# LuoweiZhou/VLP

Measured on NVIDIA H100. Metric: image_text_samples_per_sec, higher is better.
Workload: dtype bf16

## Files before the change

### vlp_b200/csrc/api.cu

```cuda
#include "../../include/vlpk.h"

#include <cstdlib>
#include <cstring>

#include "attn.cuh"
#include "decode.cuh"
#include "gemm.cuh"
#include "head.cuh"
#include "host.cuh"
#include "optim.cuh"
#include "rowops.cuh"
#include "tables.cuh"

using namespace vlpk;
typedef __nv_bfloat16 bf16;

namespace {

inline cudaStream_t S(void* s) { return reinterpret_cast<cudaStream_t>(s); }

enum { SITE_ATTN = 0, SITE_HID1 = 1, SITE_HID2 = 2 };
inline uint64_t site_of(uint64_t layer_id, int site) { return layer_id * 8 + site; }

inline DropoutCfg mk_drop(const VlpkDropout* d, float p, uint64_t site) {
// ... 187 lines not shown
  VLPK_TRY(launch_attn_fwd(ad, st));
  VLPK_TRY(fwd_linear(Mq, H, H, a->ctx, H, w->wo, H, w->bo, a->t1, H, EPI_STORE, nullptr, 0, none, st));
  LnArgs ln;
  ln.M = Mq; ln.H = H;
  ln.t = static_cast<const bf16*>(a->t1); ln.res = static_cast<const bf16*>(x);
  ln.gamma = static_cast<const bf16*>(w->ln1_g); ln.beta = static_cast<const bf16*>(w->ln1_b);
  ln.y = static_cast<bf16*>(a->y1); ln.stats = reinterpret_cast<float2*>(a->stats1);
  ln.drop = mk_drop(drop, p_hidden, site_of(layer_id, SITE_HID1));
  return launch_ln_res_drop_fwd(ln, st);
}

int ffn_fwd_impl(const VlpkShape* s, const VlpkLayerWeights* w, VlpkLayerActs* a, float p_hidden, const VlpkDropout* drop,
                 uint64_t layer_id, cudaStream_t st) {
  const int H = s->H, I = s->I, M = s->B * s->Lq;
  const DropoutCfg none = make_dropout(0.f, 0, 0);
  VLPK_TRY(fwd_linear(M, I, H, a->y1, H, w->w1, H, w->b1, a->u, I, EPI_GELU, a->hmid, I, none, st));
  VLPK_TRY(fwd_linear(M, H, I, a->hmid, I, w->w2, I, w->b2, a->t2, H, EPI_STORE, nullptr, 0, none, st));
  LnArgs ln;
  ln.M = M; ln.H = H;
  ln.t = static_cast<const bf16*>(a->t2); ln.res = static_cast<const bf16*>(a->y1);
  ln.gamma = static_cast<const bf16*>(w->ln2_g); ln.beta = static_cast<const bf16*>(w->ln2_b);
  ln.y = static_cast<bf16*>(a->y); ln.stats = reinterpret_cast<float2*>(a->stats2);
  ln.drop = mk_drop(drop, p_hidden, site_of(layer_id, SITE_HID2));
  return launch_ln_res_drop_fwd(ln, st);
}

int ffn_bwd_impl(const VlpkShape* s, const VlpkLayerWeights* w, const VlpkLayerActs* a, const void* dy, void* dy1,
                 const VlpkLayerGrads* g, const VlpkBwdScratch* ws, float p_hidden, const VlpkDropout* drop, uint64_t layer_id,
                 cudaStream_t st) {
  VLPK_CHECK_ARG(s->Lq == s->Lkv, "ffn_bwd: training path requires Lq == Lkv");
  const int H = s->H, I = s->I, M = s->B * s->Lq;
  const bool hdrop = (drop != nullptr && p_hidden > 0.f);
  LnArgs l2;
  l2.M = M; l2.H = H;
  l2.t = static_cast<const bf16*>(a->t2); l2.res = static_cast<const bf16*>(a->y1);
  l2.gamma = static_cast<const bf16*>(w->ln2_g); l2.stats = reinterpret_cast<float2*>(a->stats2);
  l2.dy = static_cast<const bf16*>(dy);
  l2.dz = static_cast<bf16*>(ws->dz2);
  l2.dt = hdrop ? static_cast<bf16*>(ws->dt2) : nullptr;
  l2.dgamma = g->ln2_g; l2.dbeta = g->ln2_b; l2.dbias = g->b2;
  l2.drop = mk_drop(drop, p_hidden, site_of(layer_id, SITE_HID2));
  VLPK_TRY(launch_ln_res_drop_bwd(l2, st));
  const void* dt2 = hdrop ? ws->dt2 : ws->dz2;
  VLPK_TRY(linear_bwd_pair(
      st, [&](cudaStream_t q) { return wgrad_linear(M, H, I, dt2, H, a->hmid, I, g->w2, I, q); },
      [&](cudaStream_t q) {
        if (!deterministic()) return dgrad_linear(M, H, I, dt2, H, w->w2, I, ws->du, I, EPI_MUL, a->u, I, q, g->b1);
        VLPK_TRY(dgrad_linear(M, H, I, dt2, H, w->w2, I, ws->du, I, EPI_MUL, a->u, I, q));
        return launch_colsum(ws->du, I, M, I, g->b1, q);
      }));
  VLPK_TRY(linear_bwd_pair(
      st, [&](cudaStream_t q) { return wgrad_linear(M, I, H, ws->du, I, a->y1, H, g->w1, H, q); },
      [&](cudaStream_t q) { return dgrad_linear(M, I, H, ws->du, I, w->w1, H, dy1, H, EPI_ADD, ws->dz2, H, q); }));
  return wgrad_join(st);
}

int mha_bwd_impl(const VlpkShape* s, const VlpkLayerWeights* w, const void* x, const uint32_t* bits, int mask_rows,
                 const VlpkLayerActs* a, const void* dy1, void* dx, const VlpkLayerGrads* g, const VlpkBwdScratch* ws, float p_attn,
                 float p_hidden, const VlpkDropout* drop, uint64_t layer_id, cudaStream_t st) {
  VLPK_CHECK_ARG(s->Lq == s->Lkv, "mha_bwd: training path requires Lq == Lkv");
  const int H = s->H, M = s->B * s->Lq;
  const bool hdrop = (drop != nullptr && p_hidden > 0.f);
  LnArgs l1;
  l1.M = M; l1.H = H;
  l1.t = static_cast<const bf16*>(a->t1); l1.res = static_cast<const bf16*>(x);
  l1.gamma = static_cast<const bf16*>(w->ln1_g); l1.stats = reinterpret_cast<float2*>(a->stats1);
  l1.dy = static_cast<const bf16*>(dy1);
  l1.dz = static_cast<bf16*>(ws->dz1);
  l1.dt = hdrop ? static_cast<bf16*>(ws->dt1) : nullptr;
  l1.dgamma = g->ln1_g; l1.dbeta = g->ln1_b; l1.dbias = g->bo;
  l1.drop = mk_drop(drop, p_hidden, site_of(layer_id, SITE_HID1));
  VLPK_TRY(launch_ln_res_drop_bwd(l1, st));
  const void* dt1 = hdrop ? ws->dt1 : ws->dz1;
  VLPK_TRY(linear_bwd_pair(
      st, [&](cudaStream_t q) { return wgrad_linear(M, H, H, dt1, H, a->ctx, H, g->wo, H, q); },
      [&](cudaStream_t q) { return dgrad_linear(M, H, H, dt1, H, w->wo, H, ws->dctx, H, EPI_STORE, nullptr, 0, q); }));
  AttnDesc ad;
  ad.B = s->B; ad.heads = s->heads; ad.Lq = s->Lq; ad.Lkv = s->Lkv; ad.kv_slots = s->kv_slots;
  ad.q = a->qkv; ad.k = static_cast<const bf16*>(a->qkv) + H; ad.v = static_cast<const bf16*>(a->qkv) + 2 * H;
  ad.ld_q = 3 * H; ad.ld_kv = 3 * H;
  ad.o = a->ctx; ad.ld_o = H; ad.d_o = ws->dctx;
  ad.mask_bits = bits; ad.mask_rows = mask_rows; ad.lse = a->lse;
  ad.dq = ws->dqkv; ad.dk = static_cast<bf16*>(ws->dqkv) + H; ad.dv = static_cast<bf16*>(ws->dqkv) + 2 * H;
  ad.ld_dqkv = 3 * H;
  ad.drop = mk_drop(drop, p_attn, site_of(layer_id, SITE_ATTN));
  if (ad.drop.p > 0.f) ad.drop.bits = a->drop_attn;
  ad.dbias = g->bqkv;
  VLPK_TRY(launch_attn_bwd(ad, st));
  GemmDesc d;
  d.M = M; d.N = H; d.K = 3 * H;
  d.A = ws->dqkv; d.lda = 3 * H;
  d.b_mn = true; d.nseg = 3; d.b_seg_rows = H; d.ldb = H;
  d.B[0] = w->wq; d.B[1] = w->wk; d.B[2] = w->wv;
  d.D0 = dx; d.ldd0 = H;
  d.epi = EPI_ADD;
  d.aux = static_cast<const bf16*>(ws->dz1); d.ld_aux = H;
  VLPK_TRY(linear_bwd_pair(
      st, [&](cudaStream_t q) { return wgrad_linear(M, 3 * H, H, ws->dqkv, 3 * H, x, H, g->wqkv, H, q); },
      [&](cudaStream_t q) { return launch_gemm(d, q); }));
  return wgrad_join(st);
}

int layer_bwd_impl(const VlpkShape* s, const VlpkLayerWeights* w, const void* x, const uint32_t* bits, int mask_rows,
                   const VlpkLayerActs* a, const void* dy, void* dx, const VlpkLayerGrads* g, const VlpkBwdScratch* ws, float p_attn,
                   float p_hidden, const VlpkDropout* drop, uint64_t layer_id, cudaStream_t st) {
  VLPK_TRY(ffn_bwd_impl(s, w, a, dy, ws->dy1, g, ws, p_hidden, drop, layer_id, st));
  return mha_bwd_impl(s, w, x, bits, mask_rows, a, ws->dy1, dx, g, ws, p_attn, p_hidden, drop, layer_id, st);
}

__global__ void add_bf16_kernel(bf16* __restrict__ dst, const bf16* __restrict__ a, const bf16* __restrict__ b, long long n) {
  const long long i = (static_cast<long long>(blockIdx.x) * blockDim.x + threadIdx.x) * 8;
  if (i + 8 <= n) {
    const uint4 ua = *reinterpret_cast<const uint4*>(a + i), ub = *reinterpret_cast<const uint4*>(b + i);
    const uint32_t wa[4] = {ua.x, ua.y, ua.z, ua.w}, wb[4] = {ub.x, ub.y, ub.z, ub.w};
    uint32_t o[4];
#pragma unroll
    for (int j = 0; j < 4; ++j) {
      const float2 x = unpack_bf16x2(wa[j]), y = unpack_bf16x2(wb[j]);
      o[j] = pack_bf16x2(x.x + y.x, x.y + y.y);
    }
    *reinterpret_cast<uint4*>(dst + i) = make_uint4(o[0], o[1], o[2], o[3]);
  } else {
    for (long long k = i; k < n; ++k) dst[k] = __float2bfloat16_rn(__bfloat162float(a[k]) + __bfloat162float(b[k]));
  }
}

__global__ void relu_bwd_kernel(bf16* __restrict__ dpre, const bf16* __restrict__ dy, const bf16* __restrict__ y, long long M,
                                int N, long long lddy, long long ldy, float scale) {
  const long long i = (static_cast<long long>(blockIdx.x) * blockDim.x + threadIdx.x) * 8;
  if (i >= M * N) return;
  const long long r = i / N;
  const int c = static_cast<int>(i % N);
  const uint4 ud = *reinterpret_cast<const uint4*>(dy + r * lddy + c), uy = *reinterpret_cast<const uint4*>(y + r * ldy + c);
  const uint32_t wd[4] = {ud.x, ud.y, ud.z, ud.w}, wy[4] = {uy.x, uy.y, uy.z, uy.w};
  uint32_t o[4];
#pragma unroll
  for (int j = 0; j < 4; ++j) {
    const float2 d = unpack_bf16x2(wd[j]), v = unpack_bf16x2(wy[j]);
    o[j] = pack_bf16x2(v.x > 0.f ? d.x * scale : 0.f, v.y > 0.f ? d.y * scale : 0.f);
  }
  *reinterpret_cast<uint4*>(dpre + i) = make_uint4(o[0], o[1], o[2], o[3]);
}

}

#pragma GCC visibility push(default)
extern "C" {

int vlpk_version(void) { return VLPK_VERSION; }
int vlpk_debug_set_option(const char* name, int value) {
  VLPK_CHECK_ARG(name != nullptr, "set_option: null name");
  if (strcmp(name, "wgrad_stream") == 0) { g_wgrad_stream = value ? 1 : 0; return 0; }
  if (strcmp(name, "attn_tiled") == 0) { set_attn_tiled(value != 0); return 0; }
  set_error("set_option: unknown option '%s'", name);
  return -1;
}
int vlpk_debug_plan_gemm(int M, int N, int K, int a_mn, int b_mn, int nseg, int seg_rows, int epi, int bn, int splits, int* out2) {
  GemmDesc g;
  g.M = M; g.N = N; g.K = K;
  g.a_mn = a_mn != 0; g.b_mn = b_mn != 0;
  g.nseg = nseg; g.b_seg_rows = seg_rows;
  g.epi = epi; g.bn = bn; g.splits = splits;
  return plan_gemm(g, &out2[0], &out2[1]);
}
void vlpk_set_reserved_sms(int n) { set_reserved_sms(n); }
void vlpk_set_deterministic(int on) { set_deterministic(on != 0); }
const char* vlpk_last_error(void) { return get_error(); }

int vlpk_mask_pack(const void* mask, int dtype, int mode, int B, int rows, int kv, int64_t stride_b, int64_t stride_r, uint32_t* out,
                   void* stream) {
  VLPK_CHECK_ARG(mask != nullptr && out != nullptr, "mask_pack: null pointer");
  return launch_mask_pack(mask, dtype, mode, B, rows, kv, stride_b, stride_r, out, S(stream));
}

int vlpk_mask_synth(const int32_t* len_b, const int32_t* mode, int len_a, int B, int L, uint32_t* out, void* stream) {
  return launch_mask_synth(len_b, mode, len_a, B, L, out, S(stream));
}

int vlpk_linear_fwd(int M, int N, int K, const void* x, int64_t ldx, const void* w, int64_t ldw, const void* bias, void* y, int64_t ldy,
                    int act, const VlpkDropout* drop, uint64_t site, void* stream) {
  VLPK_CHECK_ARG(x && w && y, "linear_fwd: null pointer");
  VLPK_CHECK_ARG(act == VLPK_ACT_NONE || act == VLPK_ACT_RELU, "linear_fwd: act %d unsupported", act);
  const DropoutCfg dc = (act == VLPK_ACT_RELU && drop != nullptr) ? mk_drop(drop, drop->p, site) : make_dropout(0.f, 0, site);
  return fwd_linear(M, N, K, x, ldx, w, ldw, bias, y, ldy, act == VLPK_ACT_RELU ? EPI_RELU : EPI_STORE, nullptr, 0, dc, S(stream));
}

int vlpk_linear_bwd(int M, int N, int K, const void* x, int64_t ldx, const void* w, int64_t ldw, const void* y, int64_t ldy,
                    const void* dy, int64_t lddy, void* dpre, void* dx, int64_t lddx, float* dw, int64_t lddw, float* db, int act,
                    float p_drop, void* stream) {
  VLPK_CHECK_ARG(x && w && dy && dw, "linear_bwd: null pointer");
  cudaStream_t st = S(stream);
  const void* g = dy;
  int64_t ldg = lddy;
  if (act == VLPK_ACT_RELU) {
    VLPK_CHECK_ARG(y != nullptr && dpre != nullptr && N % 8 == 0, "linear_bwd: relu needs y, dpre and N %% 8 == 0");
    const long long n = static_cast<long long>(M) * N;
    LaunchScope scope(CAT_MISC, 6.0 * n, st);
    relu_bwd_kernel<<<static_cast<unsigned>((n / 8 + 255) / 256), 256, 0, st>>>(static_cast<bf16*>(dpre), static_cast<const bf16*>(dy),
                                                                             static_cast<const bf16*>(y), M, N, lddy, ldy,
                                                                             p_drop > 0.f ? 1.0f / (1.0f - p_drop) : 1.0f);
    VLPK_CUDA(cudaGetLastError());
    g = dpre;
    ldg = N;
  }
  if (db != nullptr) VLPK_TRY(launch_colsum(g, ldg, M, N, db, st));
  VLPK_TRY(wgrad_linear(M, N, K, g, ldg, x, ldx, dw, lddw, st));
  if (dx != nullptr) VLPK_TRY(dgrad_linear(M, N, K, g, ldg, w, ldw, dx, lddx, EPI_STORE, nullptr, 0, st));
  return 0;
}

static EmbedArgs mk_embed(int B, int L, int H, int R, int vis_input, const int64_t* ids, const int64_t* tt, const int64_t* pos,
                          const void* word_w, const void* pos_w, const void* type_w, const void* vis, const void* vpe,
                          const void* ln_g) {
  EmbedArgs a;
  a.B = B; a.L = L; a.H = H; a.R = R; a.vis_input = vis_input;
  a.ids = reinterpret_cast<const long long*>(ids);
  a.tt = reinterpret_cast<const long long*>(tt);
  a.pos = reinterpret_cast<const long long*>(pos);
  a.word = static_cast<const bf16*>(word_w); a.posw = static_cast<const bf16*>(pos_w); a.typew = static_cast<const bf16*>(type_w);
  a.vis = static_cast<const bf16*>(vis); a.vpe = static_cast<const bf16*>(vpe);
  a.gamma = static_cast<const bf16*>(ln_g);
  return a;
}

int vlpk_embed_fwd(int B, int L, int H, int R, int vis_input, const int64_t* ids, const int64_t* token_type, const int64_t* pos,
                   const void* word_w, const void* pos_w, const void* type_w, const void* vis, const void* vis_pe, const void* ln_g,
                   const void* ln_b, void* y, float* stats, const VlpkDropout* drop, uint64_t site, void* stream) {
  VLPK_CHECK_ARG(ids && word_w && pos_w && type_w && ln_g && ln_b && y, "embed_fwd: null pointer");
  EmbedArgs a = mk_embed(B, L, H, R, vis_input, ids, token_type, pos, word_w, pos_w, type_w, vis, vis_pe, ln_g);
  a.beta = static_cast<const bf16*>(ln_b);
  a.y = static_cast<bf16*>(y);
  a.stats = reinterpret_cast<float2*>(stats);
  a.drop = mk_drop(drop, drop ? drop->p : 0.f, site);
  return launch_embed_fwd(a, S(stream));
}

int vlpk_embed_bwd(int B, int L, int H, int R, int vis_input, const int64_t* ids, const int64_t* token_type, const int64_t* pos,
                   const void* word_w, const void* pos_w, const void* type_w, const void* vis, const void* vis_pe, const void* ln_g,
                   const float* stats, const void* dy, void* dz, float* d_ln_g, float* d_ln_b, const VlpkDropout* drop, uint64_t site,
                   void* stream) {
  VLPK_CHECK_ARG(ids && word_w && pos_w && type_w && ln_g && stats && dy && dz, "embed_bwd: null pointer");
  EmbedArgs a = mk_embed(B, L, H, R, vis_input, ids, token_type, pos, word_w, pos_w, type_w, vis, vis_pe, ln_g);
  a.stats = reinterpret_cast<float2*>(const_cast<float*>(stats));
  a.dy = static_cast<const bf16*>(dy);
  a.dz = static_cast<bf16*>(dz);
  a.dgamma = d_ln_g; a.dbeta = d_ln_b;
  a.drop = mk_drop(drop, drop ? drop->p : 0.f, site);
  return launch_embed_bwd(a, S(stream));
}

int vlpk_embed_tables_bwd(int B, int L, int H, int R, int vis_input, const int64_t* ids, const int64_t* token_type, const int64_t* pos,
                          const void* dz, int V, int P, int T, void* d_word, float* word_scratch, float* d_pos, float* d_type,
                          void* stream) {
  TableGradArgs a;
  a.B = B; a.L = L; a.H = H; a.R = R; a.vis_input = vis_input;
  a.V = V; a.P = P; a.T = T;
  a.ids = reinterpret_cast<const long long*>(ids);
  a.tt = reinterpret_cast<const long long*>(token_type);
  a.pos = reinterpret_cast<const long long*>(pos);
  a.dz = static_cast<const bf16*>(dz);
  a.d_word = static_cast<bf16*>(d_word);
  a.scratch = word_scratch; a.d_pos = d_pos; a.d_type = d_type;
  return launch_embed_tables_bwd(a, S(stream));
}

int vlpk_table_rows_add(int64_t n, const int64_t* ids, const int64_t* pos, const void* rows, int H, int V, int P, float scale, void* d_word,
                        float* scratch, int32_t* owner, float* d_pos, void* stream) {
  TableRowsArgs a;
  a.n = n; a.H = H; a.V = V; a.P = P; a.scale = scale;
  a.ids = reinterpret_cast<const long long*>(ids);
  a.pos = reinterpret_cast<const long long*>(pos);
  a.rows = static_cast<const bf16*>(rows);
  a.d_word = static_cast<bf16*>(d_word);
  a.scratch = scratch; a.owner = owner; a.d_pos = d_pos;
  return launch_table_rows_add(a, S(stream));
}

int vlpk_ln_res_drop_fwd(int64_t M, int H, const void* t, const void* res, const void* gamma, const void* beta, void* y, float* stats,
                         const VlpkDropout* drop, uint64_t site, void* stream) {
  VLPK_CHECK_ARG(t && gamma && beta && y, "ln_res_drop_fwd: null pointer");
  LnArgs a;
  a.M = M; a.H = H;
  a.t = static_cast<const bf16*>(t); a.res = static_cast<const bf16*>(res);
  a.gamma = static_cast<const bf16*>(gamma); a.beta = static_cast<const bf16*>(beta);
  a.y = static_cast<bf16*>(y); a.stats = reinterpret_cast<float2*>(stats);
  a.drop = mk_drop(drop, drop ? drop->p : 0.f, site);
  return launch_ln_res_drop_fwd(a, S(stream));
}

int vlpk_ln_res_drop_bwd(int64_t M, int H, const void* t, const void* res, const void* gamma, const float* stats, const void* dy,
                         void* dz, void* dt, float* dgamma, float* dbeta, float* dbias, const VlpkDropout* drop, uint64_t site,
                         void* stream) {
  VLPK_CHECK_ARG(t && gamma && stats && dy, "ln_res_drop_bwd: null pointer");
  LnArgs a;
  a.M = M; a.H = H;
  a.t = static_cast<const bf16*>(t); a.res = static_cast<const bf16*>(res);
  a.gamma = static_cast<const bf16*>(gamma);
  a.stats = reinterpret_cast<float2*>(const_cast<float*>(stats));
  a.dy = static_cast<const bf16*>(dy);
  a.dz = static_cast<bf16*>(dz); a.dt = static_cast<bf16*>(dt);
  a.dgamma = dgamma; a.dbeta = dbeta; a.dbias = dbias;
  a.drop = mk_drop(drop, drop ? drop->p : 0.f, site);
  return launch_ln_res_drop_bwd(a, S(stream));
}

int vlpk_attn_core_fwd_wide(int B, int heads, int Lq, int Lkv, const void* q, int64_t ld_q, const void* k, const void* v, int64_t ld_kv,
// ... 278 lines not shown
```

### vlp_b200/csrc/attn.cu

```cuda
#include "attn.cuh"
#include "host.cuh"
#include "rowops.cuh"

namespace vlpk {

static constexpr int HD = 64;
static constexpr int TL = 128;
static constexpr int TILE_B = TL * 128;
static constexpr float LOG2E = 1.4426950408889634f;
static constexpr float LN2 = 0.6931471805599453f;
static constexpr int ATT_THREADS = 256;

struct AttnTmaps {
  CUtensorMap q, k, v, o;
  CUtensorMap dq, dk, dv;
};

struct AttnArgs {
  int B, heads, Lq, Lkv;
  const uint32_t* mask_bits;
  int mask_rows;
  float* lse;
  const __nv_bfloat16* o_ptr;
  const __nv_bfloat16* do_ptr;
  long long ld_o;
  DropoutCfg drop;
  unsigned char* keep_out;
  float* dbias_part;
};

__device__ __forceinline__ void sw_write_pair(uint8_t* tile, int row, int col, uint32_t v) {
  *reinterpret_cast<uint32_t*>(tile + row * 128 + (((col >> 3) ^ (row & 7)) << 4) + (col & 7) * 2) = v;
}

struct Frag {
  int fr, fc;
  __device__ __forceinline__ Frag() {
    const int t = threadIdx.x & 127, lane = threadIdx.x & 31;
    fr = (t >> 5) * 16 + (lane >> 2);
    fc = (lane & 3) * 2;
  }
};

__device__ __forceinline__ float quad_max(float v) {
  v = fmaxf(v, __shfl_xor_sync(0xffffffffu, v, 1));
  return fmaxf(v, __shfl_xor_sync(0xffffffffu, v, 2));
}
__device__ __forceinline__ float quad_sum(float v) {
  v += __shfl_xor_sync(0xffffffffu, v, 1);
  return v + __shfl_xor_sync(0xffffffffu, v, 2);
}

__device__ __forceinline__ void attn_keep_words(const DropoutCfg& d, uint64_t dseed, const uint64_t (&row_elem0)[2], uint32_t (&kw)[2][4]) {
  const int lane = threadIdx.x & 31, qi = lane & 3;
#pragma unroll
  for (int h = 0; h < 2; ++h) {
    uint32_t mine = 0xFFFFFFFFu;
    if (d.p > 0.f) {
      if (d.bits != nullptr) {
        mine = __ldg(reinterpret_cast<const uint32_t*>(d.bits + (row_elem0[h] >> 3)) + qi);
      } else {
        mine = 0;
#pragma unroll
        for (int g = 0; g < 4; ++g) mine |= dropout_keep8(dseed, d.site, (row_elem0[h] + qi * 32 + g * 8) >> 3, d.thresh16) << (8 * g);
      }
    }
#pragma unroll
    for (int w = 0; w < 4; ++w) kw[h][w] = __shfl_sync(0xffffffffu, mine, (lane & ~3) | w);
  }
}

__device__ __forceinline__ float score(float s, const uint32_t (&mw)[4], int col, int Lkv) {
  const float x = s * (0.125f * LOG2E) + (((mw[col >> 5] >> (col & 31)) & 1u) ? 0.f : -10000.0f * LOG2E);
  return col < Lkv ? x : -INFINITY;
}

__device__ __forceinline__ void load_mask_words(const AttnArgs& a, int b, int row, uint32_t (&mw)[4]) {
  const int mr = (a.mask_rows == 1) ? 0 : min(row, a.mask_rows - 1);
  const uint4 m4 = __ldg(reinterpret_cast<const uint4*>(a.mask_bits + (static_cast<size_t>(b) * a.mask_rows + mr) * 4));
  mw[0] = m4.x; mw[1] = m4.y; mw[2] = m4.z; mw[3] = m4.w;
}

struct FwdSmem {
  static constexpr int OFF_Q = 0;
  static constexpr int OFF_K = TILE_B;
  static constexpr int OFF_V = 2 * TILE_B;
  static constexpr int OFF_BAR = 3 * TILE_B;
  static constexpr int TOTAL = OFF_BAR + 16;
  static constexpr int DYN = TOTAL + 1024;
};

__global__ void __launch_bounds__(ATT_THREADS, 2) attn_fwd_kernel(const __grid_constant__ AttnTmaps tm, const AttnArgs a) {
  extern __shared__ uint8_t smem_raw[];
  uint8_t* smem = reinterpret_cast<uint8_t*>((reinterpret_cast<uintptr_t>(smem_raw) + 1023) & ~uintptr_t(1023));
  uint8_t* sQ = smem + FwdSmem::OFF_Q;
  uint8_t* sK = smem + FwdSmem::OFF_K;
  uint8_t* sV = smem + FwdSmem::OFF_V;
  uint64_t* bars = reinterpret_cast<uint64_t*>(smem + FwdSmem::OFF_BAR);
  uint64_t* bar_qk = &bars[0];
  uint64_t* bar_v = &bars[1];

  pdl_launch_dependents();
  const int h = blockIdx.x, b = blockIdx.y;
  const int tid = threadIdx.x, wg = tid >> 7;
  const Frag f;
  const int qi = tid & 3;

  if (tid == 0) {
    tma_prefetch_desc(&tm.q);
    tma_prefetch_desc(&tm.k);
    tma_prefetch_desc(&tm.v);
    tma_prefetch_desc(&tm.o);
    mbar_init(bar_qk, 1);
    mbar_init(bar_v, 1);
    fence_mbar_init();
  }
  __syncthreads();
  pdl_wait();
  if (tid == 0) {
    mbar_arrive_expect_tx(bar_qk, 2 * TILE_B);
    tma_load_3d(sQ, &tm.q, bar_qk, h * HD, 0, b);
    tma_load_3d(sK, &tm.k, bar_qk, h * HD, 0, b);
    mbar_arrive_expect_tx(bar_v, TILE_B);
    tma_load_3d(sV, &tm.v, bar_v, h * HD, 0, b);
  }

  const int row[2] = {wg * 64 + f.fr, wg * 64 + f.fr + 8};
  uint32_t mw[2][4];
  uint64_t row_elem0[2];
#pragma unroll
  for (int hh = 0; hh < 2; ++hh) {
    load_mask_words(a, b, row[hh], mw[hh]);
    row_elem0[hh] = ((static_cast<uint64_t>(b) * a.heads + h) * a.Lq + min(row[hh], a.Lq - 1)) * TL;
  }

  float s[64];
  mbar_wait(bar_qk, 0);
  {
    const uint32_t q0 = smem_u32(sQ) + wg * 8192, k0 = smem_u32(sK);
    wgmma_fence();
#pragma unroll
    for (int k = 0; k < HD / 16; ++k)
      wgmma_m64n128k16_ss<0, 0>(s, wgmma_desc_sw128(q0 + k * 32, 16, 1024), wgmma_desc_sw128(k0 + k * 32, 16, 1024), k > 0 ? 1u : 0u);
    wgmma_commit();
    wgmma_wait<0>();
    reg_fence(s);
  }
  float mx[2] = {-INFINITY, -INFINITY};
#pragma unroll
  for (int i = 0; i < 64; ++i) {
    const int hh = (i >> 1) & 1;
    s[i] = score(s[i], mw[hh], 8 * (i >> 2) + f.fc + (i & 1), a.Lkv);
    mx[hh] = fmaxf(mx[hh], s[i]);
  }
  mx[0] = quad_max(mx[0]);
  mx[1] = quad_max(mx[1]);
  uint32_t kw[2][4];
  attn_keep_words(a.drop, drop_seed(a.drop), row_elem0, kw);
  if (a.keep_out != nullptr) {
#pragma unroll
    for (int hh = 0; hh < 2; ++hh)
      if (row[hh] < a.Lq) reinterpret_cast<uint32_t*>(a.keep_out + (row_elem0[hh] >> 3))[qi] = kw[hh][qi];
  }
  float rsum[2] = {0.f, 0.f}, lsum[2] = {0.f, 0.f};
  uint32_t pa[8][4];
#pragma unroll
  for (int i = 0; i < 64; i += 2) {
    const int hh = (i >> 1) & 1, col = 8 * (i >> 2) + f.fc;
    const float x0 = fast_ex2(s[i] - mx[hh]), x1 = fast_ex2(s[i + 1] - mx[hh]);
    lsum[hh] += x0 + x1;
    const float e0 = bf16_round(x0), e1 = bf16_round(x1);
    rsum[hh] += e0 + e1;
    const uint32_t keep = kw[hh][col >> 5] >> (col & 31);
    const float p0 = (keep & 1u) ? e0 * a.drop.scale : 0.f;
    const float p1 = (keep & 2u) ? e1 * a.drop.scale : 0.f;
    pa[i >> 3][(i >> 1) & 3] = pack_bf16x2(p0, p1);
  }
#pragma unroll
  for (int hh = 0; hh < 2; ++hh) {
    rsum[hh] = quad_sum(rsum[hh]);
    lsum[hh] = quad_sum(lsum[hh]);
    if (qi == 0 && a.lse != nullptr && row[hh] < a.Lq)
      a.lse[(static_cast<size_t>(b) * a.heads + h) * a.Lq + row[hh]] = (mx[hh] + log2f(lsum[hh])) * LN2;
  }
  float o[32];
  mbar_wait(bar_v, 0);
  {
    const uint32_t v0 = smem_u32(sV);
    wgmma_fence();
#pragma unroll
    for (int k = 0; k < TL / 16; ++k) wgmma_m64n64k16_rs<1>(o, pa[k], wgmma_desc_sw128(v0 + k * 2048, 8192, 1024), k > 0 ? 1u : 0u);
    wgmma_commit();
    wgmma_wait<0>();
    reg_fence(o);
  }
  const float inv[2] = {1.0f / rsum[0], 1.0f / rsum[1]};
  uint8_t* stg = sQ + wg * 8192;
#pragma unroll
  for (int i = 0; i < 32; i += 2) {
    const int hh = (i >> 1) & 1;
    sw_write_pair(stg, f.fr + 8 * hh, 8 * (i >> 2) + f.fc, pack_bf16x2(o[i] * inv[hh], o[i + 1] * inv[hh]));
  }
  fence_proxy_async_smem();
  __syncthreads();
  if (tid == 0) {
    tma_store_3d(&tm.o, sQ, h * HD, 0, b);
    tma_store_commit();
    tma_store_wait<0>();
  }
}

struct BwdSmem {
  static constexpr int OFF_Q = 0;
  static constexpr int OFF_K = TILE_B;
  static constexpr int OFF_V = 2 * TILE_B;
  static constexpr int OFF_DO = 3 * TILE_B;
  static constexpr int OFF_PD = 4 * TILE_B;
  static constexpr int OFF_BAR = 6 * TILE_B;
  static constexpr int TOTAL = OFF_BAR + 16;
  static constexpr int DYN = TOTAL + 1024;
};

__global__ void __launch_bounds__(ATT_THREADS, 1) attn_bwd_kernel(const __grid_constant__ AttnTmaps tm, const AttnArgs a) {
  extern __shared__ uint8_t smem_raw[];
  uint8_t* smem = reinterpret_cast<uint8_t*>((reinterpret_cast<uintptr_t>(smem_raw) + 1023) & ~uintptr_t(1023));
  uint8_t* sQ = smem + BwdSmem::OFF_Q;
  uint8_t* sK = smem + BwdSmem::OFF_K;
  uint8_t* sV = smem + BwdSmem::OFF_V;
  uint8_t* sdO = smem + BwdSmem::OFF_DO;
  uint8_t* sPD = smem + BwdSmem::OFF_PD;
  uint64_t* bar_in = reinterpret_cast<uint64_t*>(smem + BwdSmem::OFF_BAR);

  pdl_launch_dependents();
  const int h = blockIdx.x, b = blockIdx.y;
  const int tid = threadIdx.x, wg = tid >> 7;
  const Frag f;

  if (tid == 0) {
    tma_prefetch_desc(&tm.q);
    tma_prefetch_desc(&tm.k);
    tma_prefetch_desc(&tm.v);
    tma_prefetch_desc(&tm.o);
    mbar_init(bar_in, 1);
    fence_mbar_init();
  }
  __syncthreads();
  pdl_wait();
  if (tid == 0) {
    mbar_arrive_expect_tx(bar_in, 4 * TILE_B);
    tma_load_3d(sQ, &tm.q, bar_in, h * HD, 0, b);
    tma_load_3d(sK, &tm.k, bar_in, h * HD, 0, b);
    tma_load_3d(sV, &tm.v, bar_in, h * HD, 0, b);
    tma_load_3d(sdO, &tm.o, bar_in, h * HD, 0, b);
  }

  const int row[2] = {wg * 64 + f.fr, wg * 64 + f.fr + 8};
  uint32_t mw[2][4];
  uint64_t row_elem0[2];
  float lse2[2];
  bool row_ok[2];
#pragma unroll
  for (int hh = 0; hh < 2; ++hh) {
    load_mask_words(a, b, row[hh], mw[hh]);
    row_elem0[hh] = ((static_cast<uint64_t>(b) * a.heads + h) * a.Lq + min(row[hh], a.Lq - 1)) * TL;
    row_ok[hh] = row[hh] < a.Lq;
    lse2[hh] = row_ok[hh] ? a.lse[(static_cast<size_t>(b) * a.heads + h) * a.Lq + row[hh]] * LOG2E : 0.f;
  }
  uint32_t kw[2][4];
  attn_keep_words(a.drop, drop_seed(a.drop), row_elem0, kw);

  float s[64], dp[64];
  mbar_wait(bar_in, 0);
  {
    const uint32_t q0 = smem_u32(sQ) + wg * 8192, k0 = smem_u32(sK), do0 = smem_u32(sdO) + wg * 8192, v0 = smem_u32(sV);
    wgmma_fence();
#pragma unroll
    for (int k = 0; k < HD / 16; ++k)
      wgmma_m64n128k16_ss<0, 0>(s, wgmma_desc_sw128(q0 + k * 32, 16, 1024), wgmma_desc_sw128(k0 + k * 32, 16, 1024), k > 0 ? 1u : 0u);
#pragma unroll
    for (int k = 0; k < HD / 16; ++k)
      wgmma_m64n128k16_ss<0, 0>(dp, wgmma_desc_sw128(do0 + k * 32, 16, 1024), wgmma_desc_sw128(v0 + k * 32, 16, 1024), k > 0 ? 1u : 0u);
    wgmma_commit();
    wgmma_wait<0>();
    reg_fence(s);
    reg_fence(dp);
  }
  float delta[2] = {0.f, 0.f};
#pragma unroll
  for (int i = 0; i < 64; ++i) {
    const int hh = (i >> 1) & 1, col = 8 * (i >> 2) + f.fc + (i & 1);
    const float p = row_ok[hh] ? fast_ex2(score(s[i], mw[hh], col, a.Lkv) - lse2[hh]) : 0.f;
    const bool kp = (kw[hh][col >> 5] >> (col & 31)) & 1u;
    const float dpm = kp ? dp[i] * a.drop.scale : 0.f;
    delta[hh] = fmaf(p, dpm, delta[hh]);
    s[i] = p;
    dp[i] = dpm;
  }
  delta[0] = quad_sum(delta[0]);
  delta[1] = quad_sum(delta[1]);
  uint32_t dsa[8][4];
#pragma unroll
  for (int i = 0; i < 64; i += 2) {
    const int hh = (i >> 1) & 1, col = 8 * (i >> 2) + f.fc;
    const uint32_t keep = kw[hh][col >> 5] >> (col & 31);
    const float p0 = (keep & 1u) ? s[i] * a.drop.scale : 0.f, p1 = (keep & 2u) ? s[i + 1] * a.drop.scale : 0.f;
    sw_write_pair(sPD + (col >> 6) * TILE_B, row[hh], col & 63, pack_bf16x2(p0, p1));
    dsa[i >> 3][(i >> 1) & 3] = pack_bf16x2(s[i] * (dp[i] - delta[hh]) * 0.125f, s[i + 1] * (dp[i + 1] - delta[hh]) * 0.125f);
  }
  fence_proxy_async_smem();
  __syncthreads();

  float dv[32];
  {
    const uint32_t p0 = smem_u32(sPD) + wg * TILE_B, do0 = smem_u32(sdO);
    wgmma_fence();
#pragma unroll
    for (int k = 0; k < TL / 16; ++k)
      wgmma_m64n64k16_ss<1, 1>(dv, wgmma_desc_sw128(p0 + k * 2048, 8192, 1024), wgmma_desc_sw128(do0 + k * 2048, 8192, 1024), k > 0 ? 1u : 0u);
    wgmma_commit();
    wgmma_wait<0>();
    reg_fence(dv);
  }
  __syncthreads();
#pragma unroll
  for (int c = 0; c < 8; ++c)
#pragma unroll
    for (int e = 0; e < 4; ++e) {
      const int hh = e & 1, col = 16 * c + 8 * (e >> 1) + f.fc;
      sw_write_pair(sPD + (col >> 6) * TILE_B, row[hh], col & 63, dsa[c][e]);
    }
  fence_proxy_async_smem();
  __syncthreads();

  float dk[32], dq[32];
  {
    const uint32_t p0 = smem_u32(sPD) + wg * TILE_B, q0 = smem_u32(sQ), k0 = smem_u32(sK);
    wgmma_fence();
#pragma unroll
    for (int k = 0; k < TL / 16; ++k)
      wgmma_m64n64k16_ss<1, 1>(dk, wgmma_desc_sw128(p0 + k * 2048, 8192, 1024), wgmma_desc_sw128(q0 + k * 2048, 8192, 1024), k > 0 ? 1u : 0u);
#pragma unroll
    for (int k = 0; k < TL / 16; ++k) wgmma_m64n64k16_rs<1>(dq, dsa[k], wgmma_desc_sw128(k0 + k * 2048, 8192, 1024), k > 0 ? 1u : 0u);
    wgmma_commit();
    wgmma_wait<0>();
    reg_fence(dk);
    reg_fence(dq);
  }
  __syncthreads();
#pragma unroll
  for (int i = 0; i < 32; i += 2) {
    const int r = wg * 64 + f.fr + 8 * ((i >> 1) & 1), col = 8 * (i >> 2) + f.fc;
    sw_write_pair(sQ, r, col, pack_bf16x2(dq[i], dq[i + 1]));
    sw_write_pair(sK, r, col, pack_bf16x2(dk[i], dk[i + 1]));
    sw_write_pair(sV, r, col, pack_bf16x2(dv[i], dv[i + 1]));
  }
  fence_proxy_async_smem();
  __syncthreads();
  if (tid == 0) {
    tma_store_3d(&tm.dq, sQ, h * HD, 0, b);
    tma_store_3d(&tm.dk, sK, h * HD, 0, b);
    tma_store_3d(&tm.dv, sV, h * HD, 0, b);
    tma_store_commit();
  }
  if (a.dbias_part != nullptr && tid < 192) {
    const int o = tid >> 6, c = tid & 63;
    const uint8_t* stg = (o == 0) ? sQ : (o == 1 ? sK : sV);
    float acc = 0.f;
#pragma unroll 8
    for (int r = 0; r < TL; ++r)
      acc += __bfloat162float(*reinterpret_cast<const __nv_bfloat16*>(stg + r * 128 + (((c >> 3) ^ (r & 7)) << 4) + (c & 7) * 2));
    a.dbias_part[static_cast<size_t>(b) * 3 * a.heads * HD + o * a.heads * HD + h * HD + c] = acc;
  }
  if (tid == 0) tma_store_wait<0>();
}

static constexpr int MAX_SLOTS = 512;
static bool g_attn_tiled = false;

void set_attn_tiled(bool on) { g_attn_tiled = on; }

struct AttnTiledArgs {
  int B, heads, Lq, Lkv;
  int slots;
  int tiles;
  const uint32_t* mask_bits;
  int mask_rows;
  float* lse;
  float* delta;
  DropoutCfg drop;
  unsigned char* keep_out;
  float* dbias_part;
};

__device__ __forceinline__ void load_mask_tile(const AttnTiledArgs& a, int b, int row, int kt, uint32_t (&mw)[4]) {
  const int mr = (a.mask_rows == 1) ? 0 : min(row, a.mask_rows - 1);
  const uint4 m4 = __ldg(reinterpret_cast<const uint4*>(a.mask_bits + (static_cast<size_t>(b) * a.mask_rows + mr) * (a.slots >> 5)) + kt);
  mw[0] = m4.x; mw[1] = m4.y; mw[2] = m4.z; mw[3] = m4.w;
}

__device__ __forceinline__ uint64_t tiled_row_elem0(const AttnTiledArgs& a, int b, int h, int row) {
  return ((static_cast<uint64_t>(b) * a.heads + h) * a.Lq + min(row, a.Lq - 1)) * a.slots;
}

__device__ __forceinline__ float staged_colsum(const uint8_t* stg, int c) {
  float acc = 0.f;
#pragma unroll 8
  for (int r = 0; r < TL; ++r)
    acc += __bfloat162float(*reinterpret_cast<const __nv_bfloat16*>(stg + r * 128 + (((c >> 3) ^ (r & 7)) << 4) + (c & 7) * 2));
  return acc;
}

struct FwdTiledSmem {
  static constexpr int OFF_Q = 0;
  static constexpr int OFF_KV = TILE_B;
  static constexpr int OFF_BAR = 5 * TILE_B;
  static constexpr int TOTAL = OFF_BAR + 24;
  static constexpr int DYN = TOTAL + 1024;
};

__global__ void __launch_bounds__(ATT_THREADS, 1) attn_fwd_tiled_kernel(const __grid_constant__ AttnTmaps tm, const AttnTiledArgs a) {
  extern __shared__ uint8_t smem_raw[];
  uint8_t* smem = reinterpret_cast<uint8_t*>((reinterpret_cast<uintptr_t>(smem_raw) + 1023) & ~uintptr_t(1023));
  uint8_t* sQ = smem + FwdTiledSmem::OFF_Q;
  uint8_t* sKV = smem + FwdTiledSmem::OFF_KV;
  uint64_t* bars = reinterpret_cast<uint64_t*>(smem + FwdTiledSmem::OFF_BAR);

  pdl_launch_dependents();
  const int h = blockIdx.x, b = blockIdx.y, q0 = blockIdx.z * TL;
  const int tid = threadIdx.x, wg = tid >> 7;
  const Frag f;
  const int qi = tid & 3;
  const int nkt = (a.Lkv + TL - 1) / TL;

  if (tid == 0) {
    tma_prefetch_desc(&tm.q);
    tma_prefetch_desc(&tm.k);
    tma_prefetch_desc(&tm.v);
    tma_prefetch_desc(&tm.o);
    for (int i = 0; i < 3; ++i) mbar_init(&bars[i], 1);
    fence_mbar_init();
  }
  __syncthreads();
  pdl_wait();
  if (tid == 0) {
    mbar_arrive_expect_tx(&bars[0], TILE_B);
    tma_load_3d(sQ, &tm.q, &bars[0], h * HD, q0, b);
    for (int kt = 0; kt < 2 && kt < nkt; ++kt) {
      mbar_arrive_expect_tx(&bars[1 + kt], 2 * TILE_B);
      tma_load_3d(sKV + kt * 2 * TILE_B, &tm.k, &bars[1 + kt], h * HD, kt * TL, b);
      tma_load_3d(sKV + kt * 2 * TILE_B + TILE_B, &tm.v, &bars[1 + kt], h * HD, kt * TL, b);
    }
  }

  const int row[2] = {q0 + wg * 64 + f.fr, q0 + wg * 64 + f.fr + 8};
  uint64_t row_elem0[2];
#pragma unroll
  for (int hh = 0; hh < 2; ++hh) row_elem0[hh] = tiled_row_elem0(a, b, h, row[hh]);
  const uint64_t dseed = drop_seed(a.drop);

  float o[32];
#pragma unroll
  for (int i = 0; i < 32; ++i) o[i] = 0.f;
  float mx[2] = {-INFINITY, -INFINITY}, rsum[2] = {0.f, 0.f}, lsum[2] = {0.f, 0.f};
  mbar_wait(&bars[0], 0);
  for (int kt = 0; kt < nkt; ++kt) {
    const int st = kt & 1;
    uint8_t* sK = sKV + st * 2 * TILE_B;
    uint8_t* sV = sK + TILE_B;
    uint32_t mw[2][4];
#pragma unroll
    for (int hh = 0; hh < 2; ++hh) load_mask_tile(a, b, row[hh], kt, mw[hh]);
    float s[64];
    mbar_wait(&bars[1 + st], (kt >> 1) & 1);
    {
      const uint32_t qa = smem_u32(sQ) + wg * 8192, k0 = smem_u32(sK);
      wgmma_fence();
#pragma unroll
      for (int k = 0; k < HD / 16; ++k)
        wgmma_m64n128k16_ss<0, 0>(s, wgmma_desc_sw128(qa + k * 32, 16, 1024), wgmma_desc_sw128(k0 + k * 32, 16, 1024), k > 0 ? 1u : 0u);
      wgmma_commit();
      wgmma_wait<0>();
      reg_fence(s);
    }
    const int lkv = a.Lkv - kt * TL;
    float tmx[2] = {-INFINITY, -INFINITY};
#pragma unroll
    for (int i = 0; i < 64; ++i) {
      const int hh = (i >> 1) & 1;
      s[i] = score(s[i], mw[hh], 8 * (i >> 2) + f.fc + (i & 1), lkv);
      tmx[hh] = fmaxf(tmx[hh], s[i]);
    }
    float alpha[2];
#pragma unroll
    for (int hh = 0; hh < 2; ++hh) {
      const float mnew = fmaxf(mx[hh], quad_max(tmx[hh]));
      alpha[hh] = fast_ex2(mx[hh] - mnew);
      mx[hh] = mnew;
      lsum[hh] *= alpha[hh];
      rsum[hh] *= alpha[hh];
    }
    uint32_t kw[2][4];
    const uint64_t tile_elem0[2] = {row_elem0[0] + kt * TL, row_elem0[1] + kt * TL};
    attn_keep_words(a.drop, dseed, tile_elem0, kw);
    if (a.keep_out != nullptr) {
#pragma unroll
      for (int hh = 0; hh < 2; ++hh)
        if (row[hh] < a.Lq) reinterpret_cast<uint32_t*>(a.keep_out + (tile_elem0[hh] >> 3))[qi] = kw[hh][qi];
    }
    uint32_t pa[8][4];
#pragma unroll
    for (int i = 0; i < 64; i += 2) {
      const int hh = (i >> 1) & 1, col = 8 * (i >> 2) + f.fc;
      const float x0 = fast_ex2(s[i] - mx[hh]), x1 = fast_ex2(s[i + 1] - mx[hh]);
      lsum[hh] += x0 + x1;
      const float e0 = bf16_round(x0), e1 = bf16_round(x1);
      rsum[hh] += e0 + e1;
      const uint32_t keep = kw[hh][col >> 5] >> (col & 31);
      const float p0 = (keep & 1u) ? e0 * a.drop.scale : 0.f;
      const float p1 = (keep & 2u) ? e1 * a.drop.scale : 0.f;
      pa[i >> 3][(i >> 1) & 3] = pack_bf16x2(p0, p1);
    }
#pragma unroll
    for (int i = 0; i < 32; ++i) o[i] *= alpha[(i >> 1) & 1];
    {
      const uint32_t v0 = smem_u32(sV);
      wgmma_fence();
// ... 308 lines not shown
  if (a.dbias_part != nullptr && tid < 2 * HD) {
    const int o = 1 + (tid >> 6), c = tid & 63;
    a.dbias_part[(static_cast<size_t>(b) * a.tiles + kt) * 3 * a.heads * HD + o * a.heads * HD + h * HD + c] =
        staged_colsum(o == 1 ? sK : sV, c);
  }
  if (tid == 0) tma_store_wait<0>();
}

static int make_seq_tmap(CUtensorMap* out, const void* base, int width, int L, int B, int64_t ld, int64_t batch_stride = 0) {
  uint64_t dims[3] = {static_cast<uint64_t>(width), static_cast<uint64_t>(L), static_cast<uint64_t>(B)};
  uint64_t strides[2] = {static_cast<uint64_t>(ld) * 2,
                         batch_stride > 0 ? static_cast<uint64_t>(batch_stride) * 2 : static_cast<uint64_t>(ld) * 2 * static_cast<uint64_t>(L)};
  uint32_t box[3] = {HD, TL, 1};
  return make_tmap(out, TM_BF16, 3, base, dims, strides, box);
}

static int check_common(const AttnDesc& d) {
  VLPK_CHECK_ARG(d.head_dim == HD, "attention: head_dim %d unsupported (only 64)", d.head_dim);
  if (d.kv_slots == 0) {
    VLPK_CHECK_ARG(d.Lq >= 1 && d.Lq <= TL && d.Lkv >= 1 && d.Lkv <= TL, "attention: Lq=%d Lkv=%d must be in [1,128]",
                   d.Lq, d.Lkv);
  } else {
    VLPK_CHECK_ARG(d.Lkv >= 1 && d.Lkv <= MAX_SLOTS && d.kv_slots == (d.Lkv + TL - 1) / TL * TL && d.Lq >= 1 && d.Lq <= d.kv_slots,
                   "attention: Lq=%d Lkv=%d kv_slots=%d (needs Lkv in [1,512], kv_slots = 128 * ceil(Lkv / 128), Lq in [1,kv_slots])",
                   d.Lq, d.Lkv, d.kv_slots);
  }
  VLPK_CHECK_ARG(d.B >= 1 && d.heads >= 1, "attention: B=%d heads=%d", d.B, d.heads);
  VLPK_CHECK_ARG(d.mask_bits != nullptr && (d.mask_rows == 1 || d.mask_rows == d.Lq), "attention: mask rows %d",
                 d.mask_rows);
  return 0;
}

static bool use_tiled(const AttnDesc& d) { return g_attn_tiled || d.Lq > TL || d.Lkv > TL; }

static AttnTiledArgs tiled_args(const AttnDesc& d) {
  AttnTiledArgs a;
  a.B = d.B; a.heads = d.heads; a.Lq = d.Lq; a.Lkv = d.Lkv;
  a.slots = d.kv_slots != 0 ? d.kv_slots : TL;
  a.tiles = (d.Lq + TL - 1) / TL;
  a.mask_bits = d.mask_bits; a.mask_rows = d.mask_rows;
  a.lse = d.lse; a.delta = nullptr;
  a.drop = d.drop;
  a.keep_out = nullptr;
  a.dbias_part = nullptr;
  return a;
}

static int launch_attn_fwd_tiled(const AttnDesc& d, const AttnTmaps& tm, cudaStream_t stream) {
  AttnTiledArgs a = tiled_args(d);
  a.keep_out = d.keep_out;
  static bool attr_set = false;
  if (!attr_set) {
    VLPK_CUDA(cudaFuncSetAttribute(attn_fwd_tiled_kernel, cudaFuncAttributeMaxDynamicSharedMemorySize, FwdTiledSmem::DYN));
    attr_set = true;
  }
  LaunchScope scope(CAT_ATTN_FWD, 4.0 * d.B * d.heads * d.Lq * d.Lkv * HD, stream);
  VLPK_CUDA(launch_ex(attn_fwd_tiled_kernel, dim3(d.heads, d.B, (d.Lq + TL - 1) / TL), dim3(ATT_THREADS), FwdTiledSmem::DYN, stream, 1, tm, a));
  return 0;
}

static int launch_attn_bwd_tiled(const AttnDesc& d, const AttnTmaps& tm, cudaStream_t stream) {
  AttnTiledArgs a = tiled_args(d);
  const long long nbias = 3LL * d.heads * HD;
  a.delta = scratch_f32(SCRATCH_ATTN_DELTA, static_cast<size_t>(d.B) * d.heads * d.Lq, stream);
  if (a.delta == nullptr) return -1;
  if (d.dbias != nullptr) {
    a.dbias_part = scratch_f32(SCRATCH_ATTN_DBIAS, static_cast<size_t>(d.B) * a.tiles * nbias, stream);
    if (a.dbias_part == nullptr) return -1;
  }
  static bool attr_set = false;
  if (!attr_set) {
    VLPK_CUDA(cudaFuncSetAttribute(attn_bwd_dq_tiled_kernel, cudaFuncAttributeMaxDynamicSharedMemorySize, BwdDqSmem::DYN));
    VLPK_CUDA(cudaFuncSetAttribute(attn_bwd_dkv_tiled_kernel, cudaFuncAttributeMaxDynamicSharedMemorySize, BwdDkvSmem::DYN));
    attr_set = true;
  }
  const double flops = 10.0 * d.B * d.heads * d.Lq * d.Lkv * HD;
  {
    LaunchScope scope(CAT_ATTN_BWD, 0.4 * flops, stream);
    VLPK_CUDA(launch_ex(attn_bwd_dq_tiled_kernel, dim3(d.heads, d.B, a.tiles), dim3(ATT_THREADS), BwdDqSmem::DYN, stream, 1, tm, a));
  }
  {
    LaunchScope scope(CAT_ATTN_BWD, 0.6 * flops, stream);
    VLPK_CUDA(launch_ex(attn_bwd_dkv_tiled_kernel, dim3(d.heads, d.B, (d.Lkv + TL - 1) / TL), dim3(ATT_THREADS), BwdDkvSmem::DYN, stream, 1,
                        tm, a));
  }
  if (d.dbias != nullptr) VLPK_TRY(launch_sum_parts(a.dbias_part, d.B * a.tiles, nbias, d.dbias, stream));
  return 0;
}

int launch_attn_fwd(const AttnDesc& d, cudaStream_t stream) {
  VLPK_TRY(check_common(d));
  const int width = d.heads * HD;
  AttnTmaps tm;
  memset(&tm, 0, sizeof(tm));
  VLPK_TRY(make_seq_tmap(&tm.q, d.q, width, d.Lq, d.B, d.ld_q));
  VLPK_TRY(make_seq_tmap(&tm.k, d.k, width, d.Lkv, d.B, d.ld_kv, d.kv_batch_stride));
  VLPK_TRY(make_seq_tmap(&tm.v, d.v, width, d.Lkv, d.B, d.ld_kv, d.kv_batch_stride));
  VLPK_TRY(make_seq_tmap(&tm.o, d.o, width, d.Lq, d.B, d.ld_o));
  tm.dq = tm.dk = tm.dv = tm.o;
  if (use_tiled(d)) return launch_attn_fwd_tiled(d, tm, stream);
  AttnArgs a;
  a.B = d.B; a.heads = d.heads; a.Lq = d.Lq; a.Lkv = d.Lkv;
  a.mask_bits = d.mask_bits; a.mask_rows = d.mask_rows;
  a.lse = d.lse; a.o_ptr = nullptr; a.do_ptr = nullptr; a.ld_o = d.ld_o;
  a.drop = d.drop;
  a.keep_out = d.keep_out;
  a.dbias_part = nullptr;
  static bool attr_set = false;
  if (!attr_set) {
    VLPK_CUDA(cudaFuncSetAttribute(attn_fwd_kernel, cudaFuncAttributeMaxDynamicSharedMemorySize, FwdSmem::DYN));
    attr_set = true;
  }
  LaunchScope scope(CAT_ATTN_FWD, 4.0 * d.B * d.heads * d.Lq * d.Lkv * HD, stream);
  VLPK_CUDA(launch_ex(attn_fwd_kernel, dim3(d.heads, d.B), dim3(ATT_THREADS), FwdSmem::DYN, stream, 1, tm, a));
  return 0;
}

int launch_attn_bwd(const AttnDesc& d, cudaStream_t stream) {
  VLPK_TRY(check_common(d));
  VLPK_CHECK_ARG(d.Lq == d.Lkv, "attention bwd: Lq must equal Lkv (training path)");
  VLPK_CHECK_ARG(d.lse != nullptr && d.d_o != nullptr && d.dq && d.dk && d.dv, "attention bwd: missing buffers");
  const int width = d.heads * HD;
  AttnTmaps tm;
  memset(&tm, 0, sizeof(tm));
  VLPK_TRY(make_seq_tmap(&tm.q, d.q, width, d.Lq, d.B, d.ld_q));
  VLPK_TRY(make_seq_tmap(&tm.k, d.k, width, d.Lkv, d.B, d.ld_kv));
  VLPK_TRY(make_seq_tmap(&tm.v, d.v, width, d.Lkv, d.B, d.ld_kv));
  VLPK_TRY(make_seq_tmap(&tm.o, d.d_o, width, d.Lq, d.B, d.ld_o));
  VLPK_TRY(make_seq_tmap(&tm.dq, d.dq, width, d.Lq, d.B, d.ld_dqkv));
  VLPK_TRY(make_seq_tmap(&tm.dk, d.dk, width, d.Lkv, d.B, d.ld_dqkv));
  VLPK_TRY(make_seq_tmap(&tm.dv, d.dv, width, d.Lkv, d.B, d.ld_dqkv));
  if (use_tiled(d)) return launch_attn_bwd_tiled(d, tm, stream);
  AttnArgs a;
  a.B = d.B; a.heads = d.heads; a.Lq = d.Lq; a.Lkv = d.Lkv;
  a.mask_bits = d.mask_bits; a.mask_rows = d.mask_rows;
  a.lse = d.lse;
  a.o_ptr = reinterpret_cast<const __nv_bfloat16*>(d.o);
  a.do_ptr = reinterpret_cast<const __nv_bfloat16*>(d.d_o);
  a.ld_o = d.ld_o;
  a.drop = d.drop;
  a.keep_out = nullptr;
  a.dbias_part = nullptr;
  const long long nbias = 3LL * d.heads * HD;
  if (d.dbias != nullptr) {
    a.dbias_part = scratch_f32(SCRATCH_ATTN_DBIAS, static_cast<size_t>(d.B) * nbias, stream);
    if (a.dbias_part == nullptr) return -1;
  }
  static bool attr_set = false;
  if (!attr_set) {
    VLPK_CUDA(cudaFuncSetAttribute(attn_bwd_kernel, cudaFuncAttributeMaxDynamicSharedMemorySize, BwdSmem::DYN));
    attr_set = true;
  }
  {
    LaunchScope scope(CAT_ATTN_BWD, 10.0 * d.B * d.heads * d.Lq * d.Lkv * HD, stream);
    VLPK_CUDA(launch_ex(attn_bwd_kernel, dim3(d.heads, d.B), dim3(ATT_THREADS), BwdSmem::DYN, stream, 1, tm, a));
  }
  if (d.dbias != nullptr) VLPK_TRY(launch_sum_parts(a.dbias_part, d.B, nbias, d.dbias, stream));
  return 0;
}

}
```

### vlp_b200/csrc/attn.cuh

```cuda
#pragma once
#include "common.cuh"

namespace vlpk {

struct AttnDesc {
  int B = 0, heads = 0, head_dim = 64;
  int Lq = 0, Lkv = 0;
  int kv_slots = 0;
  const void* q = nullptr;
  const void* k = nullptr;
  const void* v = nullptr;
  int64_t ld_q = 0, ld_kv = 0;
  int64_t kv_batch_stride = 0;
  void* o = nullptr;
  int64_t ld_o = 0;
  const uint32_t* mask_bits = nullptr;
  int mask_rows = 0;
  float* lse = nullptr;
  DropoutCfg drop = {0.f, 1.f, 0u, 0ull, 0ull, nullptr};
  unsigned char* keep_out = nullptr;
  const void* d_o = nullptr;
  void* dq = nullptr;
  void* dk = nullptr;
  void* dv = nullptr;
  int64_t ld_dqkv = 0;
  float* dbias = nullptr;
};

int launch_attn_fwd(const AttnDesc& d, cudaStream_t stream);
int launch_attn_bwd(const AttnDesc& d, cudaStream_t stream);
void set_attn_tiled(bool on);

}
```

Measured before the change: 5367.

## Make attention backward persistent with double-buffered TMA prefetch of next head

Turns the attention backward kernel into a persistent grid sized to the SM count. Each block loops over (batch, head) items and prefetches the next item's Q/K/V/dO into a second smem slot while the current item computes. The aim is to hide TMA load latency and cut per-block launch and prologue overhead. The cost is twice the input smem per block plus extra barriers, and parity bookkeeping that must stay correct across the two slots.

```diff
diff --git a/vlp_b200/csrc/api.cu b/vlp_b200/csrc/api.cu
--- a/vlp_b200/csrc/api.cu
+++ b/vlp_b200/csrc/api.cu
@@ -363,6 +363,7 @@
   VLPK_CHECK_ARG(name != nullptr, "set_option: null name");
   if (strcmp(name, "wgrad_stream") == 0) { g_wgrad_stream = value ? 1 : 0; return 0; }
   if (strcmp(name, "attn_tiled") == 0) { set_attn_tiled(value != 0); return 0; }
+  if (strcmp(name, "attn_persistent") == 0) { set_attn_persistent(value != 0); return 0; }
   set_error("set_option: unknown option '%s'", name);
   return -1;
 }
diff --git a/vlp_b200/csrc/attn.cu b/vlp_b200/csrc/attn.cu
--- a/vlp_b200/csrc/attn.cu
+++ b/vlp_b200/csrc/attn.cu
@@ -35,12 +35,19 @@
 
 struct Frag {
   int fr, fc;
-  __device__ __forceinline__ Frag() {
-    const int t = threadIdx.x & 127, lane = threadIdx.x & 31;
+  __device__ __forceinline__ Frag() : Frag(threadIdx.x) {}
+  __device__ __forceinline__ explicit Frag(int tid) {
+    const int t = tid & 127, lane = tid & 31;
     fr = (t >> 5) * 16 + (lane >> 2);
     fc = (lane & 3) * 2;
   }
 };
+
+__device__ __forceinline__ int tid_opaque() {
+  int t;
+  asm volatile("mov.u32 %0, %%tid.x;" : "=r"(t));
+  return t;
+}
 
 __device__ __forceinline__ float quad_max(float v) {
   v = fmaxf(v, __shfl_xor_sync(0xffffffffu, v, 1));
@@ -80,6 +87,10 @@
   const uint4 m4 = __ldg(reinterpret_cast<const uint4*>(a.mask_bits + (static_cast<size_t>(b) * a.mask_rows + mr) * 4));
   mw[0] = m4.x; mw[1] = m4.y; mw[2] = m4.z; mw[3] = m4.w;
 }
+
+static bool g_attn_persistent = true;
+
+void set_attn_persistent(bool on) { g_attn_persistent = on; }
 
 struct FwdSmem {
   static constexpr int OFF_Q = 0;
@@ -211,48 +222,31 @@
 }
 
 struct BwdSmem {
-  static constexpr int OFF_Q = 0;
-  static constexpr int OFF_K = TILE_B;
-  static constexpr int OFF_V = 2 * TILE_B;
-  static constexpr int OFF_DO = 3 * TILE_B;
-  static constexpr int OFF_PD = 4 * TILE_B;
-  static constexpr int OFF_BAR = 6 * TILE_B;
+  static constexpr int SLOT = 4 * TILE_B;
+  static constexpr int OFF_PD = 2 * SLOT;
+  static constexpr int OFF_BAR = OFF_PD + 2 * TILE_B;
   static constexpr int TOTAL = OFF_BAR + 16;
   static constexpr int DYN = TOTAL + 1024;
 };
 
-__global__ void __launch_bounds__(ATT_THREADS, 1) attn_bwd_kernel(const __grid_constant__ AttnTmaps tm, const AttnArgs a) {
-  extern __shared__ uint8_t smem_raw[];
-  uint8_t* smem = reinterpret_cast<uint8_t*>((reinterpret_cast<uintptr_t>(smem_raw) + 1023) & ~uintptr_t(1023));
-  uint8_t* sQ = smem + BwdSmem::OFF_Q;
-  uint8_t* sK = smem + BwdSmem::OFF_K;
-  uint8_t* sV = smem + BwdSmem::OFF_V;
-  uint8_t* sdO = smem + BwdSmem::OFF_DO;
+__device__ __forceinline__ void attn_bwd_load(const AttnTmaps& tm, uint8_t* slot, uint64_t* bar, int h, int b) {
+  mbar_arrive_expect_tx(bar, 4 * TILE_B);
+  tma_load_3d(slot, &tm.q, bar, h * HD, 0, b);
+  tma_load_3d(slot + TILE_B, &tm.k, bar, h * HD, 0, b);
+  tma_load_3d(slot + 2 * TILE_B, &tm.v, bar, h * HD, 0, b);
+  tma_load_3d(slot + 3 * TILE_B, &tm.o, bar, h * HD, 0, b);
+}
+
+__device__ __forceinline__ void attn_bwd_item(const AttnTmaps& tm, const AttnArgs& a, uint8_t* smem, int st, uint32_t par, int w, int next) {
+  uint8_t* sQ = smem + st * BwdSmem::SLOT;
+  uint8_t* sK = sQ + TILE_B;
+  uint8_t* sV = sQ + 2 * TILE_B;
+  uint8_t* sdO = sQ + 3 * TILE_B;
   uint8_t* sPD = smem + BwdSmem::OFF_PD;
-  uint64_t* bar_in = reinterpret_cast<uint64_t*>(smem + BwdSmem::OFF_BAR);
-
-  pdl_launch_dependents();
-  const int h = blockIdx.x, b = blockIdx.y;
-  const int tid = threadIdx.x, wg = tid >> 7;
-  const Frag f;
-
-  if (tid == 0) {
-    tma_prefetch_desc(&tm.q);
-    tma_prefetch_desc(&tm.k);
-    tma_prefetch_desc(&tm.v);
-    tma_prefetch_desc(&tm.o);
-    mbar_init(bar_in, 1);
-    fence_mbar_init();
-  }
-  __syncthreads();
-  pdl_wait();
-  if (tid == 0) {
-    mbar_arrive_expect_tx(bar_in, 4 * TILE_B);
-    tma_load_3d(sQ, &tm.q, bar_in, h * HD, 0, b);
-    tma_load_3d(sK, &tm.k, bar_in, h * HD, 0, b);
-    tma_load_3d(sV, &tm.v, bar_in, h * HD, 0, b);
-    tma_load_3d(sdO, &tm.o, bar_in, h * HD, 0, b);
-  }
+  uint64_t* bars = reinterpret_cast<uint64_t*>(smem + BwdSmem::OFF_BAR);
+  const int h = w % a.heads, b = w / a.heads;
+  const int tid = tid_opaque(), wg = tid >> 7;
+  const Frag f(tid);
 
   const int row[2] = {wg * 64 + f.fr, wg * 64 + f.fr + 8};
   uint32_t mw[2][4];
@@ -266,11 +260,16 @@
     row_ok[hh] = row[hh] < a.Lq;
     lse2[hh] = row_ok[hh] ? a.lse[(static_cast<size_t>(b) * a.heads + h) * a.Lq + row[hh]] * LOG2E : 0.f;
   }
+  __syncthreads();
+  if (tid == 0 && next >= 0) {
+    tma_store_wait_read<0>();
+    attn_bwd_load(tm, smem + (st ^ 1) * BwdSmem::SLOT, &bars[st ^ 1], next % a.heads, next / a.heads);
+  }
   uint32_t kw[2][4];
   attn_keep_words(a.drop, drop_seed(a.drop), row_elem0, kw);
 
   float s[64], dp[64];
-  mbar_wait(bar_in, 0);
+  mbar_wait(&bars[st], par);
   {
     const uint32_t q0 = smem_u32(sQ) + wg * 8192, k0 = smem_u32(sK), do0 = smem_u32(sdO) + wg * 8192, v0 = smem_u32(sV);
     wgmma_fence();
@@ -371,7 +370,33 @@
       acc += __bfloat162float(*reinterpret_cast<const __nv_bfloat16*>(stg + r * 128 + (((c >> 3) ^ (r & 7)) << 4) + (c & 7) * 2));
     a.dbias_part[static_cast<size_t>(b) * 3 * a.heads * HD + o * a.heads * HD + h * HD + c] = acc;
   }
-  if (tid == 0) tma_store_wait<0>();
+}
+
+__global__ void __launch_bounds__(ATT_THREADS, 1) attn_bwd_kernel(const __grid_constant__ AttnTmaps tm, const AttnArgs a) {
+  extern __shared__ uint8_t smem_raw[];
+  uint8_t* smem = reinterpret_cast<uint8_t*>((reinterpret_cast<uintptr_t>(smem_raw) + 1023) & ~uintptr_t(1023));
+  uint64_t* bars = reinterpret_cast<uint64_t*>(smem + BwdSmem::OFF_BAR);
+  const int items = a.B * a.heads;
+
+  pdl_launch_dependents();
+  if (threadIdx.x == 0) {
+    tma_prefetch_desc(&tm.q);
+    tma_prefetch_desc(&tm.k);
+    tma_prefetch_desc(&tm.v);
+    tma_prefetch_desc(&tm.o);
+    mbar_init(&bars[0], 1);
+    mbar_init(&bars[1], 1);
+    fence_mbar_init();
+  }
+  __syncthreads();
+  pdl_wait();
+  if (threadIdx.x == 0) attn_bwd_load(tm, smem, &bars[0], blockIdx.x % a.heads, blockIdx.x / a.heads);
+  for (int it = 0;; ++it) {
+    const int w = blockIdx.x + it * gridDim.x, next = w + gridDim.x;
+    if (w >= items) break;
+    attn_bwd_item(tm, a, smem, it & 1, (it >> 1) & 1, w, next < items ? next : -1);
+  }
+  if (threadIdx.x == 0) tma_store_wait<0>();
 }
 
 static constexpr int MAX_SLOTS = 512;
@@ -986,8 +1011,10 @@
     attr_set = true;
   }
   {
+    const int items = d.B * d.heads;
+    const int grid = g_attn_persistent ? std::min(items, gemm_sms()) : items;
     LaunchScope scope(CAT_ATTN_BWD, 10.0 * d.B * d.heads * d.Lq * d.Lkv * HD, stream);
-    VLPK_CUDA(launch_ex(attn_bwd_kernel, dim3(d.heads, d.B), dim3(ATT_THREADS), BwdSmem::DYN, stream, 1, tm, a));
+    VLPK_CUDA(launch_ex(attn_bwd_kernel, dim3(grid), dim3(ATT_THREADS), BwdSmem::DYN, stream, 1, tm, a));
   }
   if (d.dbias != nullptr) VLPK_TRY(launch_sum_parts(a.dbias_part, d.B, nbias, d.dbias, stream));
   return 0;
diff --git a/vlp_b200/csrc/attn.cuh b/vlp_b200/csrc/attn.cuh
--- a/vlp_b200/csrc/attn.cuh
+++ b/vlp_b200/csrc/attn.cuh
@@ -30,5 +30,6 @@
 int launch_attn_fwd(const AttnDesc& d, cudaStream_t stream);
 int launch_attn_bwd(const AttnDesc& d, cudaStream_t stream);
 void set_attn_tiled(bool on);
+void set_attn_persistent(bool on);
 
 }
```

Measured after the change: 5387 (median of 6 runs). Within noise of the previous version (+0.4%).
